# Sunshine-718/AlphaZero-AL

Hardware: AMD Instinct MI355X
Metric: self-play positions/sec (Connect4 n_playout=200, batch=8192 games/GPU, vl_batch=4) (higher is better)
Workload: dtype f32; 1 GPU; Connect4 self-play, n_playout=200, 8192 games/GPU, vl_batch=4, evaluator=cnn; c_base=1000, use_symmetry=True, lead_in_plies=12, streams_per_gpu=1, parallelism=independent game shards x1

## Files before the change

### alphazero-al_amd/csrc/engine.hip

```cpp
#include "engine_internal.h"

thread_local std::string az::host::g_last_error;

namespace {
constexpr int64_t kInitialSlots = 4096;

az_mcts *create_engine(int game, int n_envs, int device)
{
    if (!known_game(game)) throw AzError(AZ_ERR_ARG, "unknown game id");
    if (n_envs <= 0) throw AzError(AZ_ERR_ARG, "n_envs must be positive");
    int count = 0;
    const hipError_t dev_err = hipGetDeviceCount(&count);
    if (dev_err != hipSuccess || count <= 0)
        throw AzError(AZ_ERR_DEVICE, std::string("no HIP device available: the search engine runs on the GPU only (hipGetDeviceCount: ") +
                                         hipGetErrorString(dev_err) + ", " + std::to_string(count) + " devices)");
    if (device >= 0) HIP_OK(hipSetDevice(device));
    auto *m = new az_mcts();
    try {
        HIP_OK(hipGetDevice(&m->device));
        m->game = game;
        m->geo = geo_of(game);
        m->vl_leaf.max_path = m->plain_leaf.max_path = m->geo.max_path;
        m->B = n_envs;
        m->cfg.c_init = 1.25f; m->cfg.c_base = 19652.0f; m->cfg.dirichlet_alpha = 0.3f;
// ... 100 lines not shown
                   uint8_t *done, int32_t *winner, int64_t n, int reset_finished, void *stream)
{
    return guarded([&] {
        require(n >= 0, "az_c4_dev_step: negative size");
        if (n == 0) return;
        az::launch_game_step(AZ_GAME_CONNECT4, bb_p1, bb_p2, turns, nullptr, actions, done, winner, n, reset_finished != 0,
                             static_cast<hipStream_t>(stream));
    });
}

int az_game_dev_step(int game, uint64_t *bb_p1, uint64_t *bb_p2, int32_t *turns, int32_t *aux, const int32_t *actions,
                     uint8_t *done, int32_t *winner, int64_t n, int reset_finished, void *stream)
{
    return guarded([&] {
        require(known_game(game), "az_game_dev_step: unknown game");
        require(n >= 0, "az_game_dev_step: negative size");
        if (n == 0) return;
        az::launch_game_step(game, bb_p1, bb_p2, turns, aux, actions, done, winner, n, reset_finished != 0,
                             static_cast<hipStream_t>(stream));
    });
}

int az_game_dev_valid_mask(int game, const uint64_t *bb_p1, const uint64_t *bb_p2, const int32_t *turns,
                           const int32_t *aux, uint8_t *mask, int64_t n, void *stream)
{
    return guarded([&] {
        require(known_game(game), "az_game_dev_valid_mask: unknown game");
        require(n >= 0, "az_game_dev_valid_mask: negative size");
        if (n == 0) return;
        az::launch_game_valid_mask(game, bb_p1, bb_p2, turns, aux, mask, n, static_cast<hipStream_t>(stream));
    });
}

int az_mcts_max_used(az_mcts *m, int64_t *out)
{
    return guarded([&] {
        HIP_OK(hipSetDevice(m->device));
        m->flush_resets(nullptr);
        HIP_OK(hipDeviceSynchronize());
        *out = m->true_max_used();
        m->used_bound = *out;
    });
}

int az_mcts_counters(az_mcts *m, int64_t out[AZ_NUM_COUNTERS])
{
    return guarded([&] {
        HIP_OK(hipSetDevice(m->device));
        unsigned long long h[az::CNT_N * az::CNT_STRIPES];
        HIP_OK(hipDeviceSynchronize());
        HIP_OK(hipMemcpy(h, m->counters.p, sizeof h, hipMemcpyDeviceToHost));
        for (int i = 0; i < az::CNT_N; ++i) {
            unsigned long long sum = 0;
            for (int st = 0; st < az::CNT_STRIPES; ++st) sum += h[st * az::CNT_N + i];
            out[i] = static_cast<int64_t>(sum);
        }
        out[az::CNT_SELECT_LAUNCHES] = m->select_launches;
        out[az::CNT_BACKPROP_LAUNCHES] = m->backprop_launches;
        m->check_device_error();
    });
}

int az_mcts_counters_reset(az_mcts *m)
{
    return guarded([&] {
        HIP_OK(hipSetDevice(m->device));
// ... 42 lines not shown
```

### alphazero-al_amd/csrc/engine_internal.h

```cpp
#pragma once
#include <hip/hip_runtime.h>

#include <algorithm>
#include <cmath>
#include <cstdint>
#include <cstdlib>
#include <cstring>
#include <memory>
#include <stdexcept>
#include <string>
#include <vector>

#include "az_mcts.h"
#include "az_nn.h"
#include "host_rng.h"
#include "kernels.h"
#include "games.h"

namespace az::host {

extern thread_local std::string g_last_error;

struct AzError : std::runtime_error {
    int code;
// ... 370 lines not shown
        used_bound += extra;
        for (auto &g : growth_after) g += extra;
        last_extra = extra;
        growth_since_prune += extra;
    }

    void check_device_error()
    {
        int e = 0;
        HIP_OK(hipMemcpy(&e, err.p, sizeof(int), hipMemcpyDeviceToHost));
        if (e) {
            HIP_OK(hipMemset(err.p, 0, sizeof(int)));
            if (err_host) *err_host = 0;
            throw AzError(AZ_ERR_CAPACITY, device_error_text(e));
        }
    }
    static std::string device_error_text(int e)
    {
        std::string msg;
        if (e & az::ERR_ARENA_OVERFLOW) msg += "tree arena overflow on device (expansions were dropped)";
        if (e & az::ERR_LIST_OVERFLOW) msg += std::string(msg.empty() ? "" : "; ") + "compact leaf list overflow on device (entries were dropped)";
        if (msg.empty()) msg = "device error word " + std::to_string(e);
        return msg;
    }

    void prune_on(const int32_t *actions_dev, int32_t *noise_req, bool dev_noise, const float *noise_replay, hipStream_t s)
    {
        const int64_t q = ++prune_seq;
        if (ring_seq[q % 8] != 0 && live_ring[q % 8] < 0) HIP_OK(hipStreamSynchronize(s));
        live_ring[q % 8] = -1;
        ring_seq[q % 8] = q;
        growth_after[q % 8] = 0;
        HIP_OK(hipMemsetAsync(max_live.p, 0, sizeof(int), s));
        static const bool always = getenv("AZ_COMPACT_ALWAYS") != nullptr && getenv("AZ_COMPACT_ALWAYS")[0] == '1';
        const int64_t ply = std::max<int64_t>(std::max(growth_since_prune, last_extra), geo.max_edges);
        growth_since_prune = 0;
        const int64_t above = always ? 0 : std::max<int64_t>(S / 8, S - 2 * ply);
        az::launch_prune(game, arena(), params(), actions_dev, noise_req, dev_noise, s, noise_replay, max_live.p, err.p,
                         static_cast<int>(above));
        HIP_OK(hipMemcpyAsync(const_cast<int *>(&live_ring[q % 8]), max_live.p, sizeof(int), hipMemcpyDeviceToHost, s));
    }
    ~az_mcts()
    {
        if (err_host) (void)hipHostFree(err_host);
        if (live_ring) (void)hipHostFree(const_cast<int *>(live_ring));
    }
};
```

### alphazero-al_amd/csrc/kernels.h

```cpp
#pragma once

#include <hip/hip_runtime.h>

#include <cstdint>

#include "tree_layout.h"

namespace az {

struct SearchParams {
    float c_init, c_base, noise_eps, fpu_reduction, mlh_slope, mlh_cap, value_decay, alpha;
    float score_utility_factor;
    int   vl_count;
    int   use_symmetry;
    const float *cpuct_tab;
    int   tab_n;
    const float *term_aux_tab;
    uint64_t seed;
    const uint64_t *call_ptr;
    const float *noise_eps_tree;
};

struct TreeArena {
    HotRec  *hot;
// ... 43 lines not shown
constexpr int ERR_ARENA_OVERFLOW = 1;
constexpr int ERR_LIST_OVERFLOW  = 2;

enum : int { CNT_SIMS = 0, CNT_LEVELS, CNT_EXPANSIONS, CNT_TERMINAL, CNT_DUP, CNT_BACKUP,
             CNT_SELECT_LAUNCHES, CNT_BACKPROP_LAUNCHES, CNT_N };
constexpr int CNT_STRIPES = 64;
static_assert(CNT_N == 8, "one counter stripe is one 64-byte line");

void launch_import(int game, const int8_t *boards, const int32_t *turns, RootState rs, int B, hipStream_t s);
void launch_set_roots(int game, const uint64_t *bb0, const uint64_t *bb1, const int32_t *turns, RootState rs,
                      int B, hipStream_t s);
void launch_bump_call(uint64_t *call_ctr, hipStream_t s, uint64_t amount = 1);
const char *launch_select(int game, TreeArena ar, RootState rs, LeafBuf lf, SearchParams p, int K, bool vl,
                          unsigned long long *counters, hipStream_t s, uint64_t *bump_call = nullptr,
                          int64_t *zero = nullptr);
void launch_backprop(int game, TreeArena ar, LeafBuf lf, SearchParams p, int K, bool vl, bool fused,
                     EvalIn in, unsigned long long *counters, int *err, hipStream_t s);
void launch_remove_vl(int game, TreeArena ar, LeafBuf lf, SearchParams p, int K, int strideK, hipStream_t s);
void launch_export(int game, LeafBuf lf, SearchParams p, int n_leaves, bool gen_sym, int8_t *boards,
                   uint8_t *valid_mask, float *features, hipStream_t s);
void launch_prune(int game, TreeArena ar, SearchParams p, const int32_t *actions, int32_t *noise_req,
                  bool dev_noise, hipStream_t s, const float *replay_noise, int *max_live, int *err, int compact_above);
void launch_apply_noise(int game, TreeArena ar, const int32_t *noise_req, const float *noise, hipStream_t s);
void launch_reset_masked(TreeArena ar, const uint8_t *mask, hipStream_t s);
void launch_counts(int game, TreeArena ar, int32_t *counts, hipStream_t s);
void launch_root_stats(int game, TreeArena ar, float *stats, hipStream_t s);
void launch_init_trees(TreeArena ar, hipStream_t s);
void launch_rollout(int game, LeafBuf lf, SearchParams p, int B, float *policy, float *d, float *p1w, float *p2w,
                    float *ml, uint8_t *is_term, hipStream_t s);
void launch_rollout_search(int game, TreeArena ar, RootState rs, LeafBuf lf, SearchParams p, int n_sims, uint64_t call_off,
                           unsigned long long *counters, int *err, hipStream_t s);
void launch_game_step(int game, uint64_t *bb0, uint64_t *bb1, int32_t *turns, int32_t *aux, const int32_t *actions,
                      uint8_t *done, int32_t *winner, int64_t n, bool reset_finished, hipStream_t s);
void launch_game_valid_mask(int game, const uint64_t *bb0, const uint64_t *bb1, const int32_t *turns, const int32_t *aux,
                            uint8_t *mask, int64_t n, hipStream_t s);

void launch_leaf_prep(int game, LeafBuf lf, SearchParams p, int n_leaves, bool gen_sym, uint8_t *valid_mask, int32_t *idx,
                      int64_t *count, int *err, hipStream_t s);
void launch_live_leaves(LeafBuf lf, int n_leaves, int32_t *idx, int64_t *count, int *err, hipStream_t s, bool clear_count = true);
void launch_tt_lookup(int game, LeafBuf lf, int n_leaves, TtTable t, const uint64_t *clock, float *probs, float *wdl, float *ml,
                      int32_t *miss_idx, int64_t *miss_count, uint64_t *keys, int *err, hipStream_t s);
void launch_tt_insert(int game, int n_leaves, TtTable t, const uint64_t *clock, const int32_t *miss_idx, const int64_t *miss_count,
                      const uint64_t *keys, const float *probs, const float *wdl, const float *ml, hipStream_t s);

void launch_tt_refresh_gather(int game, TtTable t, uint64_t e0, int n, uint64_t *bb_p1, uint64_t *bb_p2, int32_t *turn, int32_t *sym,
                              uint8_t *mask, int32_t *rows, int64_t *count, uint64_t *keys, hipStream_t s);
void launch_tt_refresh_store(int game, TtTable t, uint64_t e0, int n, const int32_t *rows, const int64_t *count, const uint64_t *keys,
                             const float *probs, const float *wdl, const float *ml, hipStream_t s);

struct SpRows {
    uint64_t *bb0, *bb1;
    int8_t   *turn;
    float    *prob;
    float    *wdl;
    uint8_t  *mask;
};

struct SpPick {
    const int32_t *counts;
    const float   *stats;
    const int32_t *ply;
    const uint8_t *dead;
    const int32_t *tape;
    int32_t       *actions;
    const uint64_t *bb0, *bb1;
    const int32_t *turn, *aux;
// ... 109 lines not shown
```

### alphazero-al_amd/csrc/kernels.hip

```cpp
#include "tree_dev.h"

namespace az {
namespace {


template <class G>
__global__ void __launch_bounds__(256) k_import(const int8_t *boards, const int32_t *turns, RootState rs, int B)
{
    const int t = blockIdx.x * blockDim.x + threadIdx.x;
    if (t >= B) return;
    GameState s;
    s.turn = turns[t];
    G::import_cells(boards + static_cast<size_t>(t) * G::CELLS, s);
    rs.bb0[t] = s.bb0; rs.bb1[t] = s.bb1; rs.turn[t] = s.turn; rs.aux[t] = s.aux;
}

template <class G>
__global__ void __launch_bounds__(256) k_set_roots(const uint64_t *bb0, const uint64_t *bb1, const int32_t *turns,
                                                   RootState rs, int B)
{
    const int t = blockIdx.x * blockDim.x + threadIdx.x;
    if (t >= B) return;
    const uint64_t a = bb0[t], b = bb1[t];
    rs.bb0[t] = a; rs.bb1[t] = b; rs.turn[t] = turns[t];
// ... 96 lines not shown
    h.meta = META_TURN_P1 | META_EXISTS;
    hot[0] = h;
    ColdRec c;
    c.w_draw = 0.f; c.noise = 0.f; c.parent = -1; c.reserved = 0;
    cold[0] = c;
}

__global__ void __launch_bounds__(256) k_init_trees(TreeArena ar)
{
    const int t = blockIdx.x * blockDim.x + threadIdx.x;
    if (t >= ar.B) return;
    write_fresh_root(ar.hot + tree_base(ar, t), ar.cold + tree_base(ar, t));
    ar.root[t] = 0;
    ar.used[t] = 1;
}

__global__ void __launch_bounds__(256) k_reset_masked(TreeArena ar, const uint8_t *mask)
{
    const int t = blockIdx.x * blockDim.x + threadIdx.x;
    if (t >= ar.B || !mask[t]) return;
    write_fresh_root(ar.hot + tree_base(ar, t), ar.cold + tree_base(ar, t));
    ar.root[t] = 0;
    ar.used[t] = 1;
}

template <int L>
__device__ __forceinline__ unsigned long long group_ballot(bool pred, int lane)
{
    const unsigned long long bal = __ballot(pred);
    constexpr unsigned long long mask = L >= 64 ? ~0ull : ((1ull << (L & 63)) - 1ull);
    return (bal >> (lane - lane % L)) & mask;
}

template <class G>
__global__ void __launch_bounds__(WAVE) k_prune(TreeArena ar, SearchParams p, const int32_t *actions,
                                                int32_t *noise_req, int dev_noise, const float *replay_noise,
                                                int *max_live, int *err, int compact_above)
{
    const int lane = threadIdx.x;
    const int t = blockIdx.x;
    const int S = static_cast<int>(ar.S);
    const int h = ar.half[t];
    HotRec *hot = ar.hot + (static_cast<size_t>(t) * 2 + h) * ar.S;
    ColdRec *cold = ar.cold + (static_cast<size_t>(t) * 2 + h) * ar.S;
    HotRec *nhot = ar.hot + (static_cast<size_t>(t) * 2 + (1 - h)) * ar.S;
    ColdRec *ncold = ar.cold + (static_cast<size_t>(t) * 2 + (1 - h)) * ar.S;
    const int root = ar.root[t];
    const HotRec R = hot[root];
    const int action = actions[t];
    const int E = (R.meta & META_EXPANDED) ? static_cast<int>((R.meta & META_NEDGE_MASK) >> META_NEDGE_SHIFT) : 0;
    HotRec c = empty_rec();
    bool match = false;
    if (lane < E) {
        c = hot[R.child_off + lane];
        match = static_cast<int>(c.meta & META_ACTION_MASK) == action && (c.meta & META_EXISTS);
    }
    const unsigned long long mb = __ballot(match);
    if (!mb) {
        if (lane == 0) {
            write_fresh_root(hot, cold);
            ar.root[t] = 0;
            ar.used[t] = 1;
            if (!dev_noise) noise_req[t] = 0;
            atomicMax(max_live, 1);
        }
        return;
    }
    const int e = __ffsll(mb) - 1;
    const int old_root = R.child_off + e;
    if (ar.used[t] <= compact_above) {
        const uint32_t nm = static_cast<uint32_t>(__shfl(static_cast<int>(c.meta), e, WAVE));
        const int noff0 = __shfl(c.child_off, e, WAVE);
        const int nE0 = (nm & META_EXPANDED) ? static_cast<int>((nm & META_NEDGE_MASK) >> META_NEDGE_SHIFT) : 0;
        if (lane == 0) {
            ar.root[t] = old_root;
            cold[old_root].parent = -1;
            atomicMax(max_live, ar.used[t]);
        }
        const int want0 = (p.alpha > 0.0f) ? nE0 : 0;
// ... 10 lines not shown
            }
            const float sum = wave_ordered_sum(g, want0);
            if (lane < want0) cold[noff0 + lane].noise = g * (1.0f / (sum + 1e-8f));
        }
        return;
    }
    if (lane == 0) {
        nhot[0] = hot[old_root];
        ColdRec cr = cold[old_root];
        cr.parent = -1;
        ncold[0] = cr;
    }
    __builtin_amdgcn_fence(__ATOMIC_SEQ_CST, "workgroup");
    int lo = 0, hi = 1, used = 1;
    bool overflow = false;
    while (lo < hi && !overflow) {
        for (int q0 = lo; q0 < hi; q0 += WAVE) {
            const int q = q0 + lane;
            const bool valid = q < hi;
            HotRec rec = empty_rec();
            if (valid) rec = nhot[q];
            const int nE = (valid && (rec.meta & META_EXPANDED)) ? static_cast<int>((rec.meta & META_NEDGE_MASK) >> META_NEDGE_SHIFT) : 0;
            int incl = nE;
#pragma unroll
            for (int o = 1; o < WAVE; o <<= 1) {
                const int v = __shfl_up(incl, o, WAVE);
                if (lane >= o) incl += v;
            }
            const int total = __shfl(incl, WAVE - 1, WAVE);
            if (used + total > S) { overflow = true; break; }
            if (nE > 0) {
                const int dst = used + incl - nE;
                nhot[q].child_off = dst;
                for (int j = 0; j < nE; ++j) {
                    nhot[dst + j] = hot[rec.child_off + j];
                    ColdRec y = cold[rec.child_off + j];
                    y.parent = q;
                    ncold[dst + j] = y;
                }
            }
            used += total;
        }
        __builtin_amdgcn_fence(__ATOMIC_SEQ_CST, "workgroup");
        lo = hi; hi = used;
    }
    if (overflow && lane == 0) atomicOr(err, ERR_ARENA_OVERFLOW);
    const HotRec NR = nhot[0];
    const int nE = (NR.meta & META_EXPANDED) ? static_cast<int>((NR.meta & META_NEDGE_MASK) >> META_NEDGE_SHIFT) : 0;
    const int noff = NR.child_off;
    if (lane == 0) {
        ar.half[t] = static_cast<uint8_t>(1 - h);
        ar.root[t] = 0;
        ar.used[t] = used;
        atomicMax(max_live, used);
    }
    const int want = (p.alpha > 0.0f) ? nE : 0;
    if (want == 0 && lane < nE) ncold[noff + lane].noise = 0.0f;
    if (!dev_noise) {
        if (lane == 0) noise_req[t] = want;
    } else if (want > 0 && replay_noise != nullptr) {
        if (lane < want) ncold[noff + lane].noise = replay_noise[static_cast<size_t>(t) * G::ACTIONS + lane];
    } else if (want > 0) {
        float g = 0.0f;
        if (lane < want) {
            DevRng rng(p.seed, *p.call_ptr, static_cast<uint64_t>(t), static_cast<uint64_t>(lane) + 128);
            g = rng.gamma(p.alpha);
        }
        const float sum = wave_ordered_sum(g, want);
        if (lane < want) ncold[noff + lane].noise = g * (1.0f / (sum + 1e-8f));
    }
}

// ... 112 lines not shown
        code = random_playout<G>(s, p.seed, *p.call_ptr, static_cast<uint64_t>(t));
    }
    is_term[t] = term ? 1 : 0;
    d[t] = code == 0 ? 1.0f : 0.0f;
    p1w[t] = code == 1 ? 1.0f : 0.0f;
    p2w[t] = code == 2 ? 1.0f : 0.0f;
    ml[t] = 0.0f;
    for (int a = 0; a < G::ACTIONS; ++a) policy[static_cast<size_t>(t) * G::ACTIONS + a] = term ? 0.0f : 1.0f;
}


template <class G>
__global__ void __launch_bounds__(256) k_game_step(uint64_t *bb0, uint64_t *bb1, int32_t *turns, int32_t *aux,
                                                   const int32_t *actions, uint8_t *done, int32_t *winner,
                                                   int64_t n, int reset_finished)
{
    const int64_t i = static_cast<int64_t>(blockIdx.x) * blockDim.x + threadIdx.x;
    if (i >= n) return;
    const int a = actions[i];
    if (a < 0 || a >= G::ACTIONS) { done[i] = 0; winner[i] = 0; return; }
    GameState s;
    s.bb0 = bb0[i]; s.bb1 = bb1[i]; s.turn = turns[i];
    s.aux = aux != nullptr ? aux[i] : G::root_aux(s.bb0, s.bb1);
    G::step(s, a);
    const int res = G::result(s);
    const bool fin = res >= 0;
    done[i] = fin ? 1 : 0;
    winner[i] = res == 1 ? 1 : (res == 2 ? -1 : 0);
    if (fin && reset_finished) G::start(s);
    bb0[i] = s.bb0; bb1[i] = s.bb1; turns[i] = s.turn;
    if (aux != nullptr) aux[i] = s.aux;
}

template <class G>
__global__ void __launch_bounds__(256) k_game_valid_mask(const uint64_t *bb0, const uint64_t *bb1, const int32_t *turns,
                                                         const int32_t *aux, uint8_t *mask, int64_t n)
{
    const int64_t gid = static_cast<int64_t>(blockIdx.x) * blockDim.x + threadIdx.x;
    const int64_t i = gid / G::ACTIONS;
    const int a = static_cast<int>(gid - i * G::ACTIONS);
    if (i >= n) return;
    GameState s;
    s.bb0 = bb0[i]; s.bb1 = bb1[i]; s.turn = turns[i];
    s.aux = aux != nullptr ? aux[i] : G::root_aux(s.bb0, s.bb1);
    mask[gid] = G::valid_in_frame(s, 0, a) ? 1 : 0;
}

__global__ void k_bump_call(uint64_t *ctr, uint64_t amount) { *ctr += amount; }

}


void launch_import(int game, const int8_t *boards, const int32_t *turns, RootState rs, int B, hipStream_t s)
{
    AZ_DISPATCH(game, hipLaunchKernelGGL(k_import<G>, dim3((B + 255) / 256), dim3(256), 0, s, boards, turns, rs, B));
}

void launch_set_roots(int game, const uint64_t *bb0, const uint64_t *bb1, const int32_t *turns, RootState rs,
                      int B, hipStream_t s)
{
    AZ_DISPATCH(game, hipLaunchKernelGGL(k_set_roots<G>, dim3((B + 255) / 256), dim3(256), 0, s, bb0, bb1, turns, rs, B));
}

void launch_bump_call(uint64_t *call_ctr, hipStream_t s, uint64_t amount)
{
    hipLaunchKernelGGL(k_bump_call, dim3(1), dim3(1), 0, s, call_ctr, amount);
// ... 35 lines not shown
}

void launch_counts(int game, TreeArena ar, int32_t *counts, hipStream_t s)
{
    AZ_DISPATCH(game, hipLaunchKernelGGL((k_root_query<G, false>), dim3(grid_for(ar.B, WAVE / G::LANES)), dim3(WAVE), 0,
                                         s, ar, counts, static_cast<float *>(nullptr)));
}

void launch_root_stats(int game, TreeArena ar, float *stats, hipStream_t s)
{
    AZ_DISPATCH(game, hipLaunchKernelGGL((k_root_query<G, true>), dim3(grid_for(ar.B, WAVE / G::LANES)), dim3(WAVE), 0,
                                         s, ar, static_cast<int32_t *>(nullptr), stats));
}

void launch_init_trees(TreeArena ar, hipStream_t s)
{
    hipLaunchKernelGGL(k_init_trees, dim3((ar.B + 255) / 256), dim3(256), 0, s, ar);
}

void launch_rollout(int game, LeafBuf lf, SearchParams p, int B, float *policy, float *d, float *p1w, float *p2w,
                    float *ml, uint8_t *is_term, hipStream_t s)
{
    AZ_DISPATCH(game, hipLaunchKernelGGL(k_rollout<G>, dim3((B + 255) / 256), dim3(256), 0, s, lf, p, B, policy, d, p1w,
                                         p2w, ml, is_term));
}

void launch_game_step(int game, uint64_t *bb0, uint64_t *bb1, int32_t *turns, int32_t *aux, const int32_t *actions,
                      uint8_t *done, int32_t *winner, int64_t n, bool reset_finished, hipStream_t s)
{
    AZ_DISPATCH(game, hipLaunchKernelGGL(k_game_step<G>, dim3(static_cast<unsigned>((n + 255) / 256)), dim3(256), 0, s,
                                         bb0, bb1, turns, aux, actions, done, winner, n, reset_finished ? 1 : 0));
}

void launch_game_valid_mask(int game, const uint64_t *bb0, const uint64_t *bb1, const int32_t *turns, const int32_t *aux,
                            uint8_t *mask, int64_t n, hipStream_t s)
{
    AZ_DISPATCH(game, hipLaunchKernelGGL(k_game_valid_mask<G>, dim3(static_cast<unsigned>((n * G::ACTIONS + 255) / 256)),
                                         dim3(256), 0, s, bb0, bb1, turns, aux, mask, n));
}

}
```

### alphazero-al_amd/src/abi.py

```python
import ctypes as C
import os

import torch


class SearchConfig(C.Structure):
    _fields_ = [(n, C.c_float) for n in ("c_init", "c_base", "dirichlet_alpha", "noise_epsilon", "fpu_reduction", "mlh_slope",
                                         "mlh_cap", "score_utility_factor", "score_scale", "value_decay")] + \
               [("use_symmetry", C.c_uint8), ("vl_count", C.c_int32)]


class SelfPlayConfig(C.Structure):
    _fields_ = [("temperature", C.c_float), ("temp_endgame", C.c_float), ("temp_decay_moves", C.c_int32),
                ("refill", C.c_int32), ("record", C.c_int32), ("noise_steps", C.c_int32),
                ("max_finished_games", C.c_int64), ("noise_eps_init", C.c_double), ("noise_eps_min", C.c_double)]


class SelfPlayGames(C.Structure):
    _fields_ = [(n, C.c_void_p) for n in ("slot", "length", "winner", "finish_ply", "row_start", "bb_p1", "bb_p2",
                                          "turn", "prob", "wdl", "mask")]


class ReplayTensorsC(C.Structure):
    _fields_ = [(n, C.c_void_p) for n in ("state", "prob", "winner", "steps_to_end", "aux_target", "root_wdl",
# ... 137 lines not shown
    ("az_mcts_create", i32, [i32, i32, i32, P(vp)]),
    ("az_mcts_destroy", None, [vp]),
    ("az_mcts_config", P(SearchConfig), [vp]),
    ("az_mcts_num_envs", i32, [vp]),
    ("az_mcts_set_seed", i32, [vp, i32]),
    ("az_mcts_reset_env", i32, [vp, i32]),
    ("az_mcts_prune_roots", i32, [vp, vp, i64]),
    ("az_mcts_search_batch", i32, [vp, vp, vp, i64, vp, vp, vp, vp, vp, vp, vp]),
    ("az_mcts_backprop_batch", i32, [vp, vp, vp, vp, vp, vp, vp, i64]),
    ("az_mcts_remove_all_vl", i32, [vp, i32]),
    ("az_mcts_search_batch_vl", i32, [vp, i32, vp, vp, i64, vp, vp, vp, vp, vp, vp, vp, vp]),
    ("az_mcts_backprop_batch_vl", i32, [vp, i32, vp, vp, vp, vp, vp, vp, vp, i64]),
    ("az_mcts_search_rollout", i32, [vp, vp, vp, i64, i32]),
    ("az_mcts_search_rollout_dev", i32, [vp, vp, vp, i64, i32]),
    ("az_mcts_get_all_counts", i32, [vp, vp]),
    ("az_mcts_get_all_root_stats", i32, [vp, vp]),
    ("az_mcts_dev_prepare", i32, [vp, i32, i64]),
    ("az_mcts_dev_prepare_stream", i32, [vp, i32, i64, vp]),
    ("az_mcts_dev_check", i32, [vp, vp]),
    ("az_mcts_dev_replay", i32, [vp, vp, i64, i64, vp]),
    ("az_mcts_dev_set_roots", i32, [vp, vp, vp, vp, vp]),
    ("az_mcts_dev_import_roots", i32, [vp, vp, vp, vp]),
    ("az_mcts_dev_select", i32, [vp, i32, i32, vp, vp, vp]),
    ("az_mcts_dev_backprop", i32, [vp, i32, i32, vp, vp, vp, vp]),
    ("az_mcts_dev_leaves", i32, [vp, i32, vp, vp, vp, vp, vp]),
    ("az_mcts_dev_leaf_syms", i32, [vp, i32, vp, vp]),
    ("az_mcts_dev_counts", i32, [vp, vp, vp]),
    ("az_mcts_dev_root_stats", i32, [vp, vp, vp]),
    ("az_mcts_dev_prune_roots", i32, [vp, vp, vp]),
    ("az_mcts_dev_reset_masked", i32, [vp, vp, vp]),
    ("az_c4_dev_step", i32, [vp, vp, vp, vp, vp, vp, i64, i32, vp]),
    ("az_game_dev_step", i32, [i32, vp, vp, vp, vp, vp, vp, vp, i64, i32, vp]),
    ("az_game_dev_valid_mask", i32, [i32, vp, vp, vp, vp, vp, i64, vp]),
    ("az_mcts_dev_set_noise_epsilons", i32, [vp, vp]),
    ("az_mcts_dev_live_leaves", i32, [vp, i32, vp, vp, vp]),
    ("az_mcts_dev_search", i32, [vp, vp, i32, i32, i32, vp]),
    ("az_mcts_dev_search_more", i32, [vp, vp, i32, i32, i32, vp]),
    ("az_mcts_dev_rollout_search", i32, [vp, i32, i32, vp]),
    ("az_selfplay_create", i32, [vp, P(SelfPlayConfig), P(vp)]),
    ("az_selfplay_destroy", None, [vp]),
    ("az_selfplay_step", i32, [vp, vp, i32, i32, i32, i32, vp]),
    ("az_selfplay_begin_ply", i32, [vp, vp]),
    ("az_selfplay_finish_ply", i32, [vp, vp]),
    ("az_selfplay_set_action_tape", i32, [vp, vp, i64]),
    ("az_selfplay_totals", i32, [vp, P(i64 * 5)]),
    ("az_selfplay_positions", i32, [vp, vp, vp, vp, vp]),
    ("az_selfplay_finished", i32, [vp, P(i64), P(i64), P(i64)]),
    ("az_selfplay_drain", i32, [vp, P(SelfPlayGames), i64, i64]),
    ("az_selfplay_export", i32, [vp, P(ReplayTensorsC), i64, i32, i64, i64, P(SelfPlayExportInfo), P(i64), vp]),
    ("az_replay_dev_store", i32, [i32, P(SelfPlayGames), vp, vp, i64, P(ReplayTensorsC), i64, i32, vp]),
    ("az_selfplay_sample", i32, [i32, vp, vp, P(SelfPlayConfig), u64, u64, vp, i64, vp]),
    ("az_selfplay_create_teams", i32, [vp, P(SelfPlayConfig), vp, P(vp)]),
    ("az_selfplay_team_sample", i32, [i32, vp, vp, P(SelfPlayConfig), i32, i32, u64, u64, vp, vp, vp, i64, vp]),
    ("az_mcts_dev_team_root_stats", i32, [i32, vp, i32, i32, vp, i64, vp]),
    ("az_match_create", i32, [vp, vp, P(MatchConfig), P(vp)]),
    ("az_match_create_teams", i32, [vp, vp, P(MatchConfig), vp, P(vp)]),
    ("az_match_destroy", None, [vp]),
    ("az_match_set_positions", i32, [vp, vp, vp, vp]),
    ("az_match_step", i32, [vp, vp, vp, i32, i32, i32, i32, vp]),
    ("az_match_step_players", i32, [vp, vp, vp, i32, i32, i32, i32, i32, i32, vp]),
    ("az_match_begin_ply", i32, [vp, vp, P(i32)]),
    ("az_match_finish_ply", i32, [vp, vp]),
    ("az_match_set_action_tape", i32, [vp, vp, i64]),
    ("az_match_remaining", i32, [vp, P(i64)]),
    ("az_match_results", i32, [vp, vp, vp, P(i64 * 4)]),
    ("az_match_moves", i32, [vp, vp]),
# ... 123 lines not shown
```

### alphazero-al_amd/src/selfplay.py

```python

import ctypes as C

import numpy as np
import torch

from src import fused as F
from src.abi import ReplayBatchC, ReplayTensorsC, SelfPlayConfig, SelfPlayExportInfo, SelfPlayGames, SelfPlayTeams, lib as selfplay_lib
from src.MCTS_cpp import BatchedMCTS
from src.replay import ReplayBatches, ReplayTensors, SampledReplayTensors, augmented, replay_tensors_c, sample_size


def _setup_search(self, net, n_games, n_playout, vl_batch, c_init, c_base, alpha, noise_epsilon, fpu_reduction,
                  use_symmetry, mlh_slope, mlh_cap, value_decay, temperature, temp_decay_moves, temp_endgame, seed,
                  table_log2, game, score_utility_factor, score_scale):
    self.B = int(n_games)
    self.n_playout = int(n_playout)
    self.vl_batch = int(vl_batch)
    self.temperature, self.temp_decay_moves, self.temp_endgame = temperature, temp_decay_moves, temp_endgame
    if c_base is None:
        c_base = 5 * n_playout
    assert game in ("Connect4", "Othello")
    self.game = game
    self.game_id = 0 if game == "Connect4" else 1
    self.MAX_PLIES = 42 if game == "Connect4" else 126
    self.search = BatchedMCTS(self.B, c_init=c_init, c_base=c_base, alpha=alpha, n_playout=n_playout,
                              game_name=game, noise_epsilon=noise_epsilon,
                              fpu_reduction=fpu_reduction, use_symmetry=use_symmetry,
                              mlh_slope=mlh_slope, mlh_cap=mlh_cap, value_decay=value_decay,
                              score_utility_factor=score_utility_factor, score_scale=score_scale)
    self.search.seed(seed)
    self.fused = F.FusedSearch(self.search, net)
    if table_log2:
        self.fused.enable_table(table_log2)
    self.h = self.fused.h
# ... 15 lines not shown
                 noise_epsilon=0.25, fpu_reduction=0.2, use_symmetry=True, mlh_slope=0.1, mlh_cap=0.2,
                 value_decay=1.0, temperature=1.0, temp_decay_moves=20, temp_endgame=0.0, seed=0,
                 reserve_slots=None, record=False, td_steps=0, refill=True, sampler="device",
                 max_finished_games=None, table_log2=0, game="Connect4", score_utility_factor=0.0, score_scale=8.0,
                 noise_steps=0, noise_eps_min=0.1):
        _setup_search(self, net, n_games, n_playout, vl_batch, c_init, c_base, alpha, noise_epsilon, fpu_reduction,
                      use_symmetry, mlh_slope, mlh_cap, value_decay, temperature, temp_decay_moves, temp_endgame, seed,
                      table_log2, game, score_utility_factor, score_scale)
        dev = self.device
        self.gen = torch.Generator(device=dev)
        self.gen.manual_seed(int(seed))
        z = dict(device=dev)
        self.start_p1, self.start_p2 = (0, 0) if game == "Connect4" else ((1 << 28) | (1 << 35), (1 << 27) | (1 << 36))
        self.bb_p1 = torch.full((self.B,), self.start_p1, dtype=torch.int64, **z)
        self.bb_p2 = torch.full((self.B,), self.start_p2, dtype=torch.int64, **z)
        self.turn = torch.ones(self.B, dtype=torch.int32, **z)
        self.aux = torch.zeros(self.B, dtype=torch.int32, **z)
        self.ply = torch.zeros(self.B, dtype=torch.int32, **z)
        self.counts = torch.zeros((self.B, self.search.action_size), dtype=torch.int32, **z)
        self.actions = torch.zeros(self.B, dtype=torch.int32, **z)
        self.done = torch.zeros(self.B, dtype=torch.uint8, **z)
        self.winner = torch.zeros(self.B, dtype=torch.int32, **z)
        self.totals = torch.zeros(5, dtype=torch.int64, **z)
        _reserve_arenas(self, reserve_slots)
        assert sampler in ("device", "reference")
        self.sampler, self.refill, self.record, self.td_steps = sampler, bool(refill), bool(record), int(td_steps)
        self.dead = torch.zeros(self.B, dtype=torch.bool, **z)
        self.ar = torch.arange(self.B, **z)
        self._c_temp = torch.tensor(float(self.temperature), **z)
        self._c_temp_end = torch.tensor(float(self.temp_endgame), **z)
        self._c_B = torch.tensor(self.B, dtype=torch.int64, **z)
        self.max_plies_ahead = 1
        self._ply_events = []
        self.noise_steps, self.noise_eps_init, self.noise_eps_min = int(noise_steps), float(noise_epsilon), float(noise_eps_min)
        if self.noise_steps > 0:
            self.eps_tree = torch.full((self.B,), self.noise_eps_init, dtype=torch.float32, **z)
            F.check(F.lib().az_mcts_dev_set_noise_epsilons(self.h, self.eps_tree.data_ptr()))
        if self.record:
            A = self.search.action_size
            self.stats = torch.zeros((self.B, 6 + 8 * A), dtype=torch.float32, **z)
            T = self.MAX_PLIES + 2
            self.G = int(max_finished_games or max(4 * self.B, 1024))
            def rows(n):
                return dict(bb1=torch.zeros((n, T), dtype=torch.int64, **z), bb2=torch.zeros((n, T), dtype=torch.int64, **z),
                            turn=torch.zeros((n, T), dtype=torch.int8, **z), prob=torch.zeros((n, T, A), dtype=torch.float32, **z),
                            wdl=torch.zeros((n, T, 3), dtype=torch.float32, **z), mask=torch.zeros((n, T, A), dtype=torch.bool, **z))
            self.rec = rows(self.B)
            self.fin = rows(self.G + 1)
            self.fin_len = torch.zeros(self.G + 1, dtype=torch.int32, **z)
            self.fin_winner = torch.zeros(self.G + 1, dtype=torch.int32, **z)
            self.fin_slot = torch.zeros(self.G + 1, dtype=torch.int32, **z)
            self.n_finished = torch.zeros((), dtype=torch.int64, **z)
            self.n_dropped = torch.zeros((), dtype=torch.int64, **z)
            self.mask_u8 = torch.zeros((self.B, A), dtype=torch.uint8, **z)

    def _pick_actions(self):
        visits = self.counts.to(torch.float32)
        greedy = visits.argmax(dim=1)
        if self.temp_decay_moves <= 0:
            temps = torch.full((self.B,), float(self.temperature), device=self.device)
        else:
            temps = torch.where(self.ply < self.temp_decay_moves, self._c_temp, self._c_temp_end)
        hot = temps > 1e-6
        t_eff = torch.where(hot, temps, torch.ones_like(temps))
        w = visits.clamp_min(0).pow(1.0 / t_eff.unsqueeze(1))
        w = torch.where(visits > 0, w, torch.zeros_like(w))
# ... 37 lines not shown
        r["wdl"][self.ar, idx] = self.stats[:, 3:6]
        F.check(F.lib().az_game_dev_valid_mask(self.game_id, self.bb_p1.data_ptr(), self.bb_p2.data_ptr(), self.turn.data_ptr(),
                                               self.aux.data_ptr(), self.mask_u8.data_ptr(), self.B, F._stream()))
        r["mask"][self.ar, idx] = self.mask_u8.bool()

    def _record_finished(self, fin):
        idx = torch.where(fin, self.ply, torch.full_like(self.ply, self.MAX_PLIES + 1)).long()
        r = self.rec
        r["bb1"][self.ar, idx] = self.bb_p1
        r["bb2"][self.ar, idx] = self.bb_p2
        r["turn"][self.ar, idx] = self.turn.to(torch.int8)
        rank = torch.cumsum(fin.to(torch.int64), 0) - 1
        dst = self.n_finished + rank
        keep = fin & (dst < self.G)
        dst = torch.where(keep, dst, torch.full_like(dst, self.G))
        for k, v in self.fin.items():
            v.index_copy_(0, dst, r[k])
        self.fin_len.index_copy_(0, dst, self.ply)
        self.fin_winner.index_copy_(0, dst, self.winner)
        self.fin_slot.index_copy_(0, dst, self.ar.to(torch.int32))
        self.n_finished += keep.sum()
        self.n_dropped += (fin & ~keep).sum()

    def step(self):
        L = F.lib()
        s = F._stream()
        F.check(L.az_mcts_dev_set_roots(self.h, self.bb_p1.data_ptr(), self.bb_p2.data_ptr(),
                                        self.turn.data_ptr(), s))
        if self.noise_steps > 0:
            decay = (1.0 - self.ply.double() / self.noise_steps).clamp_min(0.0)
            self.eps_tree.copy_((self.noise_eps_min + (self.noise_eps_init - self.noise_eps_min) * decay).float())
        self.fused.search(self.n_playout, self.vl_batch)
        F.check(L.az_mcts_dev_counts(self.h, self.counts.data_ptr(), s))
        if self.sampler == "reference":
            self._pick_actions_reference()
        else:
            self._pick_actions()
            if not self.refill:
                self.actions.masked_fill_(self.dead, -1)
        if self.record:
            F.check(L.az_mcts_dev_root_stats(self.h, self.stats.data_ptr(), s))
            self._record_position()
        F.check(L.az_mcts_dev_prune_roots(self.h, self.actions.data_ptr(), s))
        kernel_refill = 1 if (self.refill and not self.record) else 0
        F.check(L.az_game_dev_step(self.game_id, self.bb_p1.data_ptr(), self.bb_p2.data_ptr(), self.turn.data_ptr(),
                                   self.aux.data_ptr(), self.actions.data_ptr(), self.done.data_ptr(),
                                   self.winner.data_ptr(), self.B, kernel_refill, s))
        F.check(L.az_mcts_dev_reset_masked(self.h, self.done.data_ptr(), s))
        fin_b = self.done.bool()
        fin = self.done.to(torch.int64)
        self.ply = torch.where(self.dead, self.ply, self.ply + 1)
        if self.record:
            self._record_finished(fin_b)
        if self.refill:
            if not kernel_refill:
                self.bb_p1.masked_fill_(fin_b, self.start_p1)
                self.bb_p2.masked_fill_(fin_b, self.start_p2)
                self.turn.masked_fill_(fin_b, 1)
                self.aux.masked_fill_(fin_b, 0)
            self.ply = torch.where(fin_b, torch.zeros_like(self.ply), self.ply)
        else:
            self.dead |= fin_b
        self.totals += torch.stack([self._c_B, fin.sum(),
                                    (fin * (self.winner == 1)).sum(), (fin * (self.winner == -1)).sum(),
                                    (fin * (self.winner == 0)).sum()])
        F.check(L.az_mcts_dev_check(self.h, s))
        ev = torch.cuda.Event()
        ev.record()
        self._ply_events.append(ev)
        if len(self._ply_events) > self.max_plies_ahead:
            self._ply_events.pop(0).synchronize()

    def drain(self):
        assert self.record
        n = int(self.n_finished.item())
        host = {k: v[:n].cpu().numpy() for k, v in self.fin.items()}
        lens = self.fin_len[:n].cpu().numpy()
        winners = self.fin_winner[:n].cpu().numpy()
        slots = self.fin_slot[:n].cpu().numpy()
        self.n_finished.zero_()
        return assemble_games(self.game, self.td_steps, lens, winners, slots,
                              lambda g: tuple(host[k][g] for k in ("bb1", "bb2", "turn", "prob", "wdl", "mask")))

    def read_totals(self):
        t = self.totals.cpu().tolist()
        return dict(positions=t[0], games=t[1], p1_wins=t[2], p2_wins=t[3], draws=t[4])

    def engine_counters(self):
        return F.counters(self.h)


def drain_native(L, handle, action_size):
    n, rows, dropped = C.c_int64(), C.c_int64(), C.c_int64()
    F.check(L.az_selfplay_finished(handle, C.byref(n), C.byref(rows), C.byref(dropped)))
    n, rows, A = n.value, rows.value, int(action_size)
    per_game = dict(slot=np.zeros(n, np.int32), length=np.zeros(n, np.int32), winner=np.zeros(n, np.int32),
                    finish_ply=np.zeros(n, np.int64), row_start=np.zeros(n, np.int64))
    per_row = dict(bb_p1=np.zeros(rows, np.uint64), bb_p2=np.zeros(rows, np.uint64), turn=np.zeros(rows, np.int8),
                   prob=np.zeros((rows, A), np.float32), wdl=np.zeros((rows, 3), np.float32), mask=np.zeros((rows, A), np.uint8))
    out = SelfPlayGames(**{k: v.ctypes.data for k, v in list(per_game.items()) + list(per_row.items())})
    F.check(L.az_selfplay_drain(handle, C.byref(out), n, rows))
    return per_game, per_row


# ... 265 lines not shown
```

### include/az_mcts.h

```cpp
#ifndef AZ_MCTS_H
#define AZ_MCTS_H

#include <stdint.h>

#ifdef __cplusplus
extern "C" {
#endif

#define AZ_OK            0
#define AZ_ERR_ARG       1
#define AZ_ERR_DEVICE    2
#define AZ_ERR_CAPACITY  3
#define AZ_ERR_STATE     4

#define AZ_GAME_CONNECT4 0
#define AZ_GAME_OTHELLO  1

typedef struct az_search_config {
    float   c_init;
    float   c_base;
    float   dirichlet_alpha;
    float   noise_epsilon;
    float   fpu_reduction;
    float   mlh_slope;
// ... 44 lines not shown
int az_mcts_search_rollout_dev(az_mcts *m, const int8_t *boards, const int32_t *turns, int64_t n,
                               int n_playout);
int az_mcts_get_all_counts(az_mcts *m, int32_t *out);
int az_mcts_get_all_root_stats(az_mcts *m, float *out);


int az_mcts_dev_prepare(az_mcts *m, int K, int64_t sims_per_tree);
int az_mcts_dev_prepare_stream(az_mcts *m, int K, int64_t sims_per_tree, void *stream);
int az_mcts_dev_check(az_mcts *m, void *stream);
int az_mcts_dev_replay(az_mcts *m, const int32_t *sym_ids, int64_t sym_stride, int64_t n_select_calls,
                       const float *root_noise);
int az_mcts_dev_set_roots(az_mcts *m, const uint64_t *bb_p1, const uint64_t *bb_p2,
                          const int32_t *turns, void *stream);
int az_mcts_dev_import_roots(az_mcts *m, const int8_t *boards, const int32_t *turns, void *stream);
int az_mcts_dev_select(az_mcts *m, int K, int vl, float *features, uint8_t *valid_mask,
                       void *stream);
int az_mcts_dev_backprop(az_mcts *m, int K, int vl, const float *probs, const float *wdl_rel,
                         const float *moves_left, void *stream);
int az_mcts_dev_leaves(az_mcts *m, int K, uint64_t *bb_p1, uint64_t *bb_p2, int32_t *turns,
                       uint8_t *flags, void *stream);
int az_mcts_dev_leaf_syms(az_mcts *m, int K, int32_t *sym_ids, void *stream);
int az_mcts_dev_counts(az_mcts *m, int32_t *counts, void *stream);
int az_mcts_dev_root_stats(az_mcts *m, float *stats, void *stream);
int az_mcts_dev_prune_roots(az_mcts *m, const int32_t *actions, void *stream);
int az_mcts_dev_reset_masked(az_mcts *m, const uint8_t *mask, void *stream);

int az_c4_dev_step(uint64_t *bb_p1, uint64_t *bb_p2, int32_t *turns, const int32_t *actions,
                   uint8_t *done, int32_t *winner, int64_t n, int reset_finished, void *stream);
int az_game_dev_step(int game, uint64_t *bb_p1, uint64_t *bb_p2, int32_t *turns, int32_t *aux,
                     const int32_t *actions, uint8_t *done, int32_t *winner, int64_t n, int reset_finished,
                     void *stream);
int az_game_dev_valid_mask(int game, const uint64_t *bb_p1, const uint64_t *bb_p2, const int32_t *turns,
                           const int32_t *aux, uint8_t *mask, int64_t n, void *stream);

int az_mcts_dev_set_noise_epsilons(az_mcts *m, const float *per_tree);

int az_mcts_dev_live_leaves(az_mcts *m, int K, int32_t *leaf_idx, int64_t *leaf_count, void *stream);

struct az_nn_model;
int az_mcts_dev_search(az_mcts *m, const struct az_nn_model *model, int n_playout, int K, int use_table,
                       void *stream);
int az_mcts_dev_search_more(az_mcts *m, const struct az_nn_model *model, int n_sims, int K, int use_table,
                            void *stream);

int az_mcts_dev_rollout_search(az_mcts *m, int n_playout, int sims_per_launch, void *stream);

typedef struct az_selfplay_config {
    float   temperature;
    float   temp_endgame;
    int32_t temp_decay_moves;
    int32_t refill;
    int32_t record;
    int32_t noise_steps;
    int64_t max_finished_games;
    double  noise_eps_init;
    double  noise_eps_min;
} az_selfplay_config;
#define AZ_SELFPLAY_CONFIG_BYTES 48
#ifdef __cplusplus
static_assert(sizeof(az_selfplay_config) == AZ_SELFPLAY_CONFIG_BYTES, "az_selfplay_config layout");
#else
_Static_assert(sizeof(az_selfplay_config) == AZ_SELFPLAY_CONFIG_BYTES, "az_selfplay_config layout");
#endif

typedef struct az_selfplay az_selfplay;

// ... 168 lines not shown
```

Before: 308,300 positions/s.

## Fuse per-ply action pick and game advance into native kernels, vectorize prune copy

Replaces the torch-op sequence that samples moves from visit counts with one kernel that uses exponential-race sampling, and replaces the step, reset and totals bookkeeping with one fused advance kernel that resets finished trees and reduces win/draw counts with wave ballots. The prune kernel's per-child record copy becomes an unrolled dwordx4 block copy with restrict pointers. The intent is to cut many small kernel launches and Python overhead per ply and to speed up tree compaction. The risk is that the native paths differ subtly from the torch reference, for example in RNG stream use or dead-game handling, and are gated by an env var.

Result: faster. 313,000 positions/s (median of 6 runs) (+1.5%).

```diff
diff --git a/alphazero-al_amd/csrc/engine.hip b/alphazero-al_amd/csrc/engine.hip
--- a/alphazero-al_amd/csrc/engine.hip
+++ b/alphazero-al_amd/csrc/engine.hip
@@ -156,6 +156,31 @@
     });
 }
 
+int az_game_dev_pick(int game, const int32_t *counts, const float *q, const int32_t *ply, const uint8_t *dead,
+                     int32_t *actions, int64_t n, int temp_decay_moves, int hot_early, int hot_late, void *stream)
+{
+    return guarded([&] {
+        require(known_game(game), "az_game_dev_pick: unknown game");
+        require(n >= 0 && n <= INT32_MAX, "az_game_dev_pick: size out of range");
+        require(counts && q && ply && actions, "az_game_dev_pick: null array");
+        if (n == 0) return;
+        az::launch_ply_pick(game, counts, q, ply, dead, actions, static_cast<int>(n), temp_decay_moves, hot_early != 0,
+                            hot_late != 0, static_cast<hipStream_t>(stream));
+    });
+}
+
+int az_mcts_dev_ply_advance(az_mcts *m, uint64_t *bb_p1, uint64_t *bb_p2, int32_t *turns, int32_t *aux,
+                            const int32_t *actions, uint8_t *done, int32_t *winner, int32_t *ply, uint8_t *dead,
+                            int64_t *totals, int refill, void *stream)
+{
+    return guarded([&] {
+        require(bb_p1 && bb_p2 && turns && aux && actions && done && winner && ply && dead && totals,
+                "az_mcts_dev_ply_advance: null array");
+        az::launch_ply_advance(m->game, m->arena(), bb_p1, bb_p2, turns, aux, actions, done, winner, ply, dead, totals,
+                               refill != 0, static_cast<hipStream_t>(stream));
+    });
+}
+
 int az_mcts_max_used(az_mcts *m, int64_t *out)
 {
     return guarded([&] {
diff --git a/alphazero-al_amd/csrc/engine_internal.h b/alphazero-al_amd/csrc/engine_internal.h
--- a/alphazero-al_amd/csrc/engine_internal.h
+++ b/alphazero-al_amd/csrc/engine_internal.h
@@ -426,7 +426,8 @@
         ring_seq[q % 8] = q;
         growth_after[q % 8] = 0;
         HIP_OK(hipMemsetAsync(max_live.p, 0, sizeof(int), s));
-        static const bool always = getenv("AZ_COMPACT_ALWAYS") != nullptr && getenv("AZ_COMPACT_ALWAYS")[0] == '1';
+        const char *const env_always = getenv("AZ_COMPACT_ALWAYS");
+        const bool always = env_always != nullptr && env_always[0] == '1';
         const int64_t ply = std::max<int64_t>(std::max(growth_since_prune, last_extra), geo.max_edges);
         growth_since_prune = 0;
         const int64_t above = always ? 0 : std::max<int64_t>(S / 8, S - 2 * ply);
diff --git a/alphazero-al_amd/csrc/kernels.h b/alphazero-al_amd/csrc/kernels.h
--- a/alphazero-al_amd/csrc/kernels.h
+++ b/alphazero-al_amd/csrc/kernels.h
@@ -99,6 +99,11 @@
                            unsigned long long *counters, int *err, hipStream_t s);
 void launch_game_step(int game, uint64_t *bb0, uint64_t *bb1, int32_t *turns, int32_t *aux, const int32_t *actions,
                       uint8_t *done, int32_t *winner, int64_t n, bool reset_finished, hipStream_t s);
+void launch_ply_pick(int game, const int32_t *counts, const float *q, const int32_t *ply, const uint8_t *dead,
+                     int32_t *actions, int n, int decay_moves, bool hot_early, bool hot_late, hipStream_t s);
+void launch_ply_advance(int game, TreeArena ar, uint64_t *bb0, uint64_t *bb1, int32_t *turns, int32_t *aux,
+                        const int32_t *actions, uint8_t *done, int32_t *winner, int32_t *ply, uint8_t *dead,
+                        int64_t *totals, bool refill, hipStream_t s);
 void launch_game_valid_mask(int game, const uint64_t *bb0, const uint64_t *bb1, const int32_t *turns, const int32_t *aux,
                             uint8_t *mask, int64_t n, hipStream_t s);
 
diff --git a/alphazero-al_amd/csrc/kernels.hip b/alphazero-al_amd/csrc/kernels.hip
--- a/alphazero-al_amd/csrc/kernels.hip
+++ b/alphazero-al_amd/csrc/kernels.hip
@@ -152,6 +152,35 @@
     return (bal >> (lane - lane % L)) & mask;
 }
 
+template <int CH>
+__device__ __forceinline__ void copy_child_block(const HotRec *__restrict__ hot, const ColdRec *__restrict__ cold,
+                                                 HotRec *__restrict__ nhot, ColdRec *__restrict__ ncold, int src, int dst,
+                                                 int nE, int q)
+{
+    typedef uint4 __attribute__((may_alias)) rec4;
+    static_assert(sizeof(HotRec) == 2 * sizeof(rec4) && sizeof(ColdRec) == sizeof(rec4) && offsetof(ColdRec, parent) == 8,
+                  "records as dwordx4, parent in .z");
+    for (int j0 = 0; j0 < nE; j0 += CH) {
+        const rec4 *hs = reinterpret_cast<const rec4 *>(hot + src + j0);
+        const rec4 *cs = reinterpret_cast<const rec4 *>(cold + src + j0);
+        rec4 *hd = reinterpret_cast<rec4 *>(nhot + dst + j0);
+        rec4 *cd = reinterpret_cast<rec4 *>(ncold + dst + j0);
+        const int m = nE - j0;
+        uint4 ha[CH], hb[CH], cb[CH];
+#pragma unroll
+        for (int k = 0; k < CH; ++k) {
+            ha[k] = hb[k] = cb[k] = make_uint4(0u, 0u, 0u, 0u);
+            if (k < m) { ha[k] = hs[2 * k]; hb[k] = hs[2 * k + 1]; cb[k] = cs[k]; }
+        }
+#pragma unroll
+        for (int k = 0; k < CH; ++k)
+            if (k < m) {
+                cb[k].z = static_cast<unsigned>(q);
+                hd[2 * k] = ha[k]; hd[2 * k + 1] = hb[k]; cd[k] = cb[k];
+            }
+    }
+}
+
 template <class G>
 __global__ void __launch_bounds__(WAVE) k_prune(TreeArena ar, SearchParams p, const int32_t *actions,
                                                 int32_t *noise_req, int dev_noise, const float *replay_noise,
@@ -161,10 +190,10 @@
     const int t = blockIdx.x;
     const int S = static_cast<int>(ar.S);
     const int h = ar.half[t];
-    HotRec *hot = ar.hot + (static_cast<size_t>(t) * 2 + h) * ar.S;
-    ColdRec *cold = ar.cold + (static_cast<size_t>(t) * 2 + h) * ar.S;
-    HotRec *nhot = ar.hot + (static_cast<size_t>(t) * 2 + (1 - h)) * ar.S;
-    ColdRec *ncold = ar.cold + (static_cast<size_t>(t) * 2 + (1 - h)) * ar.S;
+    HotRec *__restrict__ hot = ar.hot + (static_cast<size_t>(t) * 2 + h) * ar.S;
+    ColdRec *__restrict__ cold = ar.cold + (static_cast<size_t>(t) * 2 + h) * ar.S;
+    HotRec *__restrict__ nhot = ar.hot + (static_cast<size_t>(t) * 2 + (1 - h)) * ar.S;
+    ColdRec *__restrict__ ncold = ar.cold + (static_cast<size_t>(t) * 2 + (1 - h)) * ar.S;
     const int root = ar.root[t];
     const HotRec R = hot[root];
     const int action = actions[t];
@@ -241,12 +270,7 @@
             if (nE > 0) {
                 const int dst = used + incl - nE;
                 nhot[q].child_off = dst;
-                for (int j = 0; j < nE; ++j) {
-                    nhot[dst + j] = hot[rec.child_off + j];
-                    ColdRec y = cold[rec.child_off + j];
-                    y.parent = q;
-                    ncold[dst + j] = y;
-                }
+                copy_child_block<(G::ACTIONS < 8 ? G::ACTIONS : 8)>(hot, cold, nhot, ncold, rec.child_off, dst, nE, q);
             }
             used += total;
         }
@@ -425,6 +449,85 @@
     if (aux != nullptr) aux[i] = s.aux;
 }
 
+
+template <class G>
+__global__ void __launch_bounds__(256) k_ply_pick(const int32_t *__restrict__ counts, const float *__restrict__ q,
+                                                  const int32_t *__restrict__ ply, const uint8_t *__restrict__ dead,
+                                                  int32_t *__restrict__ actions, int n, int decay_moves, int hot_early,
+                                                  int hot_late)
+{
+    constexpr int A = G::ACTIONS;
+    const int i = blockIdx.x * blockDim.x + threadIdx.x;
+    if (i >= n) return;
+    if (dead != nullptr && dead[i]) { actions[i] = -1; return; }
+    const int32_t *c = counts + static_cast<size_t>(i) * A;
+    const float *e = q + static_cast<size_t>(i) * A;
+    bool any = false;
+    int greedy = 0, gbest = c[0];
+    for (int a = 0; a < A; ++a) {
+        const int v = c[a];
+        any = any || v > 0;
+        if (v > gbest) { gbest = v; greedy = a; }
+    }
+    int sampled = 0;
+    float sbest = 0.0f;
+    for (int a = 0; a < A; ++a) {
+        const int v = c[a];
+        const float w = any ? (v > 0 ? static_cast<float>(v) : 0.0f) : 1.0f;
+        const float r = __fdiv_rn(w, e[a]);
+        if (a == 0 || r > sbest) { sbest = r; sampled = a; }
+    }
+    const bool hot = (decay_moves <= 0 || ply[i] < decay_moves) ? hot_early != 0 : hot_late != 0;
+    actions[i] = hot ? sampled : greedy;
+}
+
+template <class G>
+__global__ void __launch_bounds__(256) k_ply_advance(TreeArena ar, uint64_t *bb0, uint64_t *bb1, int32_t *turns,
+                                                     int32_t *aux, const int32_t *actions, uint8_t *done,
+                                                     int32_t *winner, int32_t *ply, uint8_t *dead,
+                                                     unsigned long long *totals, int n, int refill)
+{
+    __shared__ int s_cnt[4][4];
+    const int i = blockIdx.x * blockDim.x + threadIdx.x;
+    const int lane = threadIdx.x & 63, wave = threadIdx.x >> 6;
+    bool fin = false;
+    int w = 0;
+    if (i < n) {
+        const int a = actions[i];
+        if (a >= 0 && a < G::ACTIONS) {
+            GameState s;
+            s.bb0 = bb0[i]; s.bb1 = bb1[i]; s.turn = turns[i]; s.aux = aux[i];
+            G::step(s, a);
+            const int res = G::result(s);
+            fin = res >= 0;
+            w = res == 1 ? 1 : (res == 2 ? -1 : 0);
+            if (fin && refill) G::start(s);
+            bb0[i] = s.bb0; bb1[i] = s.bb1; turns[i] = s.turn; aux[i] = s.aux;
+        }
+        done[i] = fin ? 1 : 0;
+        winner[i] = w;
+        const bool was_dead = dead[i] != 0;
+        int pl = ply[i] + (was_dead ? 0 : 1);
+        if (fin) {
+            write_fresh_root(ar.hot + tree_base(ar, i), ar.cold + tree_base(ar, i));
+            ar.root[i] = 0;
+            ar.used[i] = 1;
+            if (refill) pl = 0; else dead[i] = 1;
+        }
+        ply[i] = pl;
+    }
+    const int c0 = __popcll(__ballot(fin)), c1 = __popcll(__ballot(fin && w == 1));
+    const int c2 = __popcll(__ballot(fin && w == -1)), c3 = __popcll(__ballot(fin && w == 0));
+    if (lane == 0) { s_cnt[wave][0] = c0; s_cnt[wave][1] = c1; s_cnt[wave][2] = c2; s_cnt[wave][3] = c3; }
+    __syncthreads();
+    if (threadIdx.x < 4) {
+        const int k = threadIdx.x;
+        const int sum = s_cnt[0][k] + s_cnt[1][k] + s_cnt[2][k] + s_cnt[3][k];
+        if (sum) atomicAdd(totals + 1 + k, static_cast<unsigned long long>(sum));
+    }
+    if (blockIdx.x == 0 && threadIdx.x == 4) atomicAdd(totals, static_cast<unsigned long long>(n));
+}
+
 template <class G>
 __global__ void __launch_bounds__(256) k_game_valid_mask(const uint64_t *bb0, const uint64_t *bb1, const int32_t *turns,
                                                          const int32_t *aux, uint8_t *mask, int64_t n)
@@ -526,6 +629,22 @@
                                          bb0, bb1, turns, aux, actions, done, winner, n, reset_finished ? 1 : 0));
 }
 
+void launch_ply_pick(int game, const int32_t *counts, const float *q, const int32_t *ply, const uint8_t *dead,
+                     int32_t *actions, int n, int decay_moves, bool hot_early, bool hot_late, hipStream_t s)
+{
+    AZ_DISPATCH(game, hipLaunchKernelGGL(k_ply_pick<G>, dim3((n + 255) / 256), dim3(256), 0, s, counts, q, ply, dead,
+                                         actions, n, decay_moves, hot_early ? 1 : 0, hot_late ? 1 : 0));
+}
+
+void launch_ply_advance(int game, TreeArena ar, uint64_t *bb0, uint64_t *bb1, int32_t *turns, int32_t *aux,
+                        const int32_t *actions, uint8_t *done, int32_t *winner, int32_t *ply, uint8_t *dead,
+                        int64_t *totals, bool refill, hipStream_t s)
+{
+    AZ_DISPATCH(game, hipLaunchKernelGGL(k_ply_advance<G>, dim3((ar.B + 255) / 256), dim3(256), 0, s, ar, bb0, bb1,
+                                         turns, aux, actions, done, winner, ply, dead,
+                                         reinterpret_cast<unsigned long long *>(totals), ar.B, refill ? 1 : 0));
+}
+
 void launch_game_valid_mask(int game, const uint64_t *bb0, const uint64_t *bb1, const int32_t *turns, const int32_t *aux,
                             uint8_t *mask, int64_t n, hipStream_t s)
 {
diff --git a/alphazero-al_amd/src/abi.py b/alphazero-al_amd/src/abi.py
--- a/alphazero-al_amd/src/abi.py
+++ b/alphazero-al_amd/src/abi.py
@@ -193,6 +193,8 @@
     ("az_c4_dev_step", i32, [vp, vp, vp, vp, vp, vp, i64, i32, vp]),
     ("az_game_dev_step", i32, [i32, vp, vp, vp, vp, vp, vp, vp, i64, i32, vp]),
     ("az_game_dev_valid_mask", i32, [i32, vp, vp, vp, vp, vp, i64, vp]),
+    ("az_game_dev_pick", i32, [i32, vp, vp, vp, vp, vp, i64, i32, i32, i32, vp]),
+    ("az_mcts_dev_ply_advance", i32, [vp, vp, vp, vp, vp, vp, vp, vp, vp, vp, vp, i32, vp]),
     ("az_mcts_dev_set_noise_epsilons", i32, [vp, vp]),
     ("az_mcts_dev_live_leaves", i32, [vp, i32, vp, vp, vp]),
     ("az_mcts_dev_search", i32, [vp, vp, i32, i32, i32, vp]),
diff --git a/alphazero-al_amd/src/selfplay.py b/alphazero-al_amd/src/selfplay.py
--- a/alphazero-al_amd/src/selfplay.py
+++ b/alphazero-al_amd/src/selfplay.py
@@ -1,5 +1,7 @@
 
 import ctypes as C
+import math
+import os
 
 import numpy as np
 import torch
@@ -81,6 +83,17 @@
         self._c_B = torch.tensor(self.B, dtype=torch.int64, **z)
         self.max_plies_ahead = 1
         self._ply_events = []
+        tail = os.environ.get("AZ_PLY_TAIL", "1") != "0"
+        t_early, t_late = np.float32(self.temperature), np.float32(self.temp_endgame)
+        self._hot_early = bool(t_early > np.float32(1e-6))
+        self._hot_late = bool(t_late > np.float32(1e-6)) if self.temp_decay_moves > 0 else self._hot_early
+        plain = float(self.temperature) == 1.0 and (self.temp_decay_moves <= 0 or not self._hot_late
+                                                    or float(self.temp_endgame) == 1.0)
+        self._native_pick = tail and sampler == "device" and plain
+        self._native_advance = tail and not self.record
+        if self._native_pick:
+            self._q = torch.empty((self.B, self.search.action_size), dtype=torch.float32, **z)
+            self._decay_moves = int(math.ceil(self.temp_decay_moves))
         self.noise_steps, self.noise_eps_init, self.noise_eps_min = int(noise_steps), float(noise_epsilon), float(noise_eps_min)
         if self.noise_steps > 0:
             self.eps_tree = torch.full((self.B,), self.noise_eps_init, dtype=torch.float32, **z)
@@ -184,7 +197,12 @@
             self.eps_tree.copy_((self.noise_eps_min + (self.noise_eps_init - self.noise_eps_min) * decay).float())
         self.fused.search(self.n_playout, self.vl_batch)
         F.check(L.az_mcts_dev_counts(self.h, self.counts.data_ptr(), s))
-        if self.sampler == "reference":
+        if self._native_pick:
+            self._q.exponential_(1.0, generator=self.gen)
+            F.check(L.az_game_dev_pick(self.game_id, self.counts.data_ptr(), self._q.data_ptr(), self.ply.data_ptr(),
+                                       None if self.refill else self.dead.data_ptr(), self.actions.data_ptr(), self.B,
+                                       self._decay_moves, int(self._hot_early), int(self._hot_late), s))
+        elif self.sampler == "reference":
             self._pick_actions_reference()
         else:
             self._pick_actions()
@@ -194,6 +212,22 @@
             F.check(L.az_mcts_dev_root_stats(self.h, self.stats.data_ptr(), s))
             self._record_position()
         F.check(L.az_mcts_dev_prune_roots(self.h, self.actions.data_ptr(), s))
+        if self._native_advance:
+            F.check(L.az_mcts_dev_ply_advance(self.h, self.bb_p1.data_ptr(), self.bb_p2.data_ptr(), self.turn.data_ptr(),
+                                              self.aux.data_ptr(), self.actions.data_ptr(), self.done.data_ptr(),
+                                              self.winner.data_ptr(), self.ply.data_ptr(), self.dead.data_ptr(),
+                                              self.totals.data_ptr(), int(self.refill), s))
+        else:
+            self._advance_torch(s)
+        F.check(L.az_mcts_dev_check(self.h, s))
+        ev = torch.cuda.Event()
+        ev.record()
+        self._ply_events.append(ev)
+        if len(self._ply_events) > self.max_plies_ahead:
+            self._ply_events.pop(0).synchronize()
+
+    def _advance_torch(self, s):
+        L = F.lib()
         kernel_refill = 1 if (self.refill and not self.record) else 0
         F.check(L.az_game_dev_step(self.game_id, self.bb_p1.data_ptr(), self.bb_p2.data_ptr(), self.turn.data_ptr(),
                                    self.aux.data_ptr(), self.actions.data_ptr(), self.done.data_ptr(),
@@ -216,12 +250,6 @@
         self.totals += torch.stack([self._c_B, fin.sum(),
                                     (fin * (self.winner == 1)).sum(), (fin * (self.winner == -1)).sum(),
                                     (fin * (self.winner == 0)).sum()])
-        F.check(L.az_mcts_dev_check(self.h, s))
-        ev = torch.cuda.Event()
-        ev.record()
-        self._ply_events.append(ev)
-        if len(self._ply_events) > self.max_plies_ahead:
-            self._ply_events.pop(0).synchronize()
 
     def drain(self):
         assert self.record
diff --git a/include/az_mcts.h b/include/az_mcts.h
--- a/include/az_mcts.h
+++ b/include/az_mcts.h
@@ -100,6 +100,12 @@
                      void *stream);
 int az_game_dev_valid_mask(int game, const uint64_t *bb_p1, const uint64_t *bb_p2, const int32_t *turns,
                            const int32_t *aux, uint8_t *mask, int64_t n, void *stream);
+
+int az_game_dev_pick(int game, const int32_t *counts, const float *q, const int32_t *ply, const uint8_t *dead,
+                     int32_t *actions, int64_t n, int temp_decay_moves, int hot_early, int hot_late, void *stream);
+int az_mcts_dev_ply_advance(az_mcts *m, uint64_t *bb_p1, uint64_t *bb_p2, int32_t *turns, int32_t *aux,
+                            const int32_t *actions, uint8_t *done, int32_t *winner, int32_t *ply, uint8_t *dead,
+                            int64_t *totals, int refill, void *stream);
 
 int az_mcts_dev_set_noise_epsilons(az_mcts *m, const float *per_tree);
 
```
